# qzwlecr/p1

Measured on AMD Instinct MI355X. Metric: SHA-256 nonce-hashes/sec (GH/s), higher is better.
Workload: dtype u32

## Files before the change

p1_amd/csrc/p1hip.hip:

```cpp
#include <hip/hip_runtime.h>
#include <rccl/rccl.h>

#include <stdlib.h>
#include <string.h>

#include <algorithm>
#include <atomic>
#include <chrono>
#include <condition_variable>
#include <exception>
#include <mutex>
#include <string>
#include <thread>
#include <utility>
#include <vector>

#include "../../include/p1hip.h"
#include "async_slots.hpp"
#include "batch_plan.hpp"
#include "below_plan.hpp"
#include "belowb_plan.hpp"
#include "planner.hpp"
#include "scan_abi.hpp"
#include "scan_pack.hpp"
#include "tile_map.hpp"
#include "wide_plan.hpp"

extern "C" const unsigned char p1hip_kernels_co[];
extern "C" const unsigned char p1hip_batch_co[];
extern "C" const unsigned char p1hip_below_co[];
extern "C" const unsigned char p1hip_belowb_co[];

using namespace p1;

namespace {

thread_local std::string g_err;

int fail(int rc, const std::string& what) {
  g_err = what;
  return rc;
}

template <typename Fn>
int guarded(Fn&& fn) {
  try {
    return fn();
  } catch (const std::exception& ex) {
    return fail(P1HIP_ERR_HIP, std::string("host: ") + ex.what());
  } catch (...) {
    return fail(P1HIP_ERR_HIP, "host: unknown exception");
  }
}

#define HIPCHK(expr)                                                                        \
  do {                                                                                      \
    hipError_t e_ = (expr);                                                                 \
    if (e_ != hipSuccess)                                                                   \
      return fail(P1HIP_ERR_HIP, std::string(#expr) + ": " + hipGetErrorString(e_));       \
  } while (0)

#define NCCLCHK(expr)                                                                       \
  do {                                                                                      \
    ncclResult_t r_ = (expr);                                                               \
    if (r_ != ncclSuccess)                                                                  \
      return fail(P1HIP_ERR_RCCL, std::string(#expr) + ": " + ncclGetErrorString(r_));      \
  } while (0)

constexpr size_t kMaxKwTabs = 8;
constexpr uint64_t kMaxKwTabBytes = 8ull << 30;
constexpr uint64_t kMaxScanSpan = 1ull << 40;

enum KnobKind { kValue, kZeroDef, kFlag };
enum KnobWhen { kPerScan, kPerBatch, kAtInit };
enum KnobId {
  kSmallMaxNoncesKnob, kMaxLaunchBlocksKnob, kMaxScanSpanKnob, kKwtabMaxBytesKnob, kNoRcclKnob, kForceRcclKnob,
  kMinFastThreadsKnob, kTestFailDeviceKnob, kNoTableKnob, kNoSplitKnob, kScanGridKnob, kBatchMaxNoncesKnob,
  kBatchMaxTilesKnob, kWideMaxNoncesKnob, kWideMaxSegsKnob, kWideMinFastThreadsKnob, kBelowPathKnob,
  kBelowMaxSliceKnob, kKnobCount
};
struct Knob {
  const char* name;
  uint64_t def, max;
  KnobKind kind;
  KnobWhen when;
  const char* what;
};
const Knob kKnobs[] = {
    {"P1HIP_SMALL_MAX_NONCES", kSmallMaxNonces, kSmallMaxNonces, kValue, kPerScan,
     "shares of at most this many nonces take the one-launch small path; 0 turns it off, so small parity ranges "
     "run the fast kernel variants"},
    {"P1HIP_MAX_LAUNCH_BLOCKS", kMaxLaunchBlocks, kMaxLaunchBlocks, kZeroDef, kPerScan,
     "workgroups per k_scan launch, so GPU tests run the multi-launch path on small ranges; a larger piece gets "
     "a launch of its own (at most kMaxFastThreads / kBlock = 2^18 workgroups, far below HIP's grid limit)"},
    {"P1HIP_MAX_SCAN_SPAN", kMaxScanSpan, ~0ull, kZeroDef, kPerScan, "nonces per piece of a device's share"},
    {"P1HIP_KWTAB_MAX_BYTES", kMaxKwTabBytes, ~0ull, kValue, kPerScan,
     "MODE 5 table cap; a larger table re-plans the share without MODE 5"},
    {"P1HIP_NO_RCCL", 0, 1, kFlag, kAtInit,
     "combine the per-device results through the host, so the multi-device path (threads, sharding, combine) "
     "runs with the same GPU listed twice on a 1-GPU box"},
    {"P1HIP_FORCE_RCCL", 0, 1, kFlag, kAtInit, "a communicator even for one device"},
    {"P1HIP_MIN_FAST_THREADS", kMinFastThreads, ~0ull, kValue, kAtInit,
     "planner occupancy floor; 1 keeps k = 3 on small ranges so every k = 3 variant runs on the GPU"},
    {"P1HIP_TEST_FAIL_DEVICE", ~0ull, ~0ull, kValue, kAtInit,
     "device index whose scan phase reports a failure (the multi-device error path); default -1: none"},
    {"P1HIP_NO_TABLE", 0, 1, kFlag, kAtInit,
     "no MODE 5: layouts whose tail block 1 holds only lo digits run the digit-update variants (A/B, and a "
     "second kernel path to cross-check MODE 5)"},
    {"P1HIP_NO_SPLIT", 0, 1, kFlag, kAtInit,
     "straddling lo digits use mode 2 instead of the split modes (A/B builds with -DP1_NV2_PLAIN)"},
    {"P1HIP_SCAN_GRID", 0, kMaxLaunchBlocks, kZeroDef, kPerScan,
     "k_scan's grid instead of the device's workgroup slots (the default, 0); at or above a launch's tile count "
     "every workgroup runs one tile and the queue hands out none (the round-5 dispatch, same code object)"},
    {"P1HIP_BATCH_MAX_NONCES", kBatchMaxNonces, kBatchMaxNonces, kValue, kPerBatch,
     "requests of at most this many nonces are coalesced by p1hip_scan_batch; 0 runs every request "
     "individually; independent of P1HIP_SMALL_MAX_NONCES"},
    {"P1HIP_BATCH_MAX_TILES", kBatchMaxTiles, kBatchMaxTiles, kZeroDef, kPerBatch,
     "tiles per launch pair, so GPU tests run several launch pairs on small batches (batch_layout raises it to "
     "the largest single request's tile count)"},
    {"P1HIP_WIDE_MAX_NONCES", kWideMaxNonces, kWideMaxNonces, kValue, kPerBatch,
     "requests above the coalescing limit and of at most this many nonces share k_scan launches in "
     "p1hip_scan_batch_wide; larger ones run individually (0: all of them)"},
    {"P1HIP_WIDE_MAX_SEGS", kMaxSegs, kMaxSegs, kZeroDef, kPerBatch,
     "segments per k_scan launch of p1hip_scan_batch_wide, so GPU tests run many launches back to back on small "
     "calls and requests whose pieces land in different launches"},
    {"P1HIP_WIDE_MIN_FAST_THREADS", 0, ~0ull, kZeroDef, kPerBatch,
     "occupancy floor the wide requests are planned with instead of wide_min_fast_threads' rule (the default, "
     "0); 1 keeps k = 3"},
    {"P1HIP_BELOW_PATH", kBelowAuto, kBelowDense, kValue, kPerScan,
     "route of every slice of p1hip_scan_below: 0 chosen from the target (the default), 1 sparse (k_scan filters, "
     "the surviving tiles are marked), 2 dense (every nonce is marked), so GPU tests run both on one range"},
    {"P1HIP_BELOW_MAX_SLICE", 0, ~0ull, kZeroDef, kPerScan,
     "nonces per slice of p1hip_scan_below at the most, below the route's own limit, so GPU tests run several "
     "slices, with hits next to their edges, on small ranges"},
};
static_assert(sizeof kKnobs / sizeof kKnobs[0] == kKnobCount, "one row per KnobId, in its order");

bool test_knobs_on() {
  const char* m = getenv("P1HIP_TEST_KNOBS");
  return m && m[0] == '1' && m[1] == 0;
}

const char* test_knob(const char* name) {
  if (!test_knobs_on()) return nullptr;
  const char* v = getenv(name);
  return v && *v ? v : nullptr;
}

uint64_t knob(KnobId id) {
  const Knob& K = kKnobs[id];
  const char* v = test_knob(K.name);
  if (!v) return K.def;
  if (K.kind == kFlag) return v[0] == '1';
  const uint64_t n = strtoull(v, nullptr, 10);
  if (n == 0 && K.kind == kZeroDef) return K.def;
  return n < K.max ? n : K.max;
}

template <typename T, bool kPinned>
struct Buf {
  T* p = nullptr;
  size_t cap = 0;

  Buf() = default;
  Buf(const Buf&) = delete;
  Buf(Buf&& o) noexcept : p(std::exchange(o.p, nullptr)), cap(std::exchange(o.cap, 0)) {}
  Buf& operator=(Buf&& o) noexcept {
    if (this != &o) {
      (void)release();
      p = std::exchange(o.p, nullptr);
      cap = std::exchange(o.cap, 0);
    }
    return *this;
  }
  ~Buf() { (void)release(); }

  hipError_t release() {
    hipError_t e = hipSuccess;
    if (p) e = kPinned ? hipHostFree(p) : hipFree(p);
    p = nullptr;
    cap = 0;
    return e;
  }
  hipError_t reserve(size_t need, size_t floor, size_t extra = 0) {
    if (need <= cap) return hipSuccess;
    hipError_t e = release();
    if (e != hipSuccess) return e;
    size_t n = floor;
    while (n < need) n <<= 1;
    const size_t bytes = (n + extra) * sizeof(T);
    e = kPinned ? hipHostMalloc(&p, bytes, hipHostMallocDefault) : hipMalloc(&p, bytes);
    if (e != hipSuccess) p = nullptr;
    else cap = n;
    return e;
  }
};
template <typename T> using DevBuf = Buf<T, false>;
template <typename T> using PinnedBuf = Buf<T, true>;

struct SlotDev {
  DevBuf<BatchSeg> d_bseg;
  PinnedBuf<BatchSeg> h_bseg;
  DevBuf<uint32_t> d_btile0;
  PinnedBuf<uint32_t> h_btile0;
  DevBuf<Key> d_bout;
  PinnedBuf<Key> h_bout;
  DevBuf<Key> d_bpart;
  DevBuf<Key> d_part;
  DevBuf<Segment> d_seg;
  PinnedBuf<Segment> h_seg;
  DevBuf<BatchSeg> d_gseg;
  PinnedBuf<BatchSeg> h_gseg;
  DevBuf<WideRange> d_wrange;
  PinnedBuf<WideRange> h_wrange;
  DevBuf<uint32_t> d_wrange0;
  PinnedBuf<uint32_t> h_wrange0;
  DevBuf<Key> d_wout;
// ... 312 lines not shown

int run_small(Dev& d, const uint8_t* msg, size_t len, uint64_t lo, uint64_t hi, bool to_host, bool profiling,
              TileDump* dump = nullptr) {
  HIPCHK(hipSetDevice(d.ordinal));
  d.ctr = {};
  Plan plan;
  std::string err = make_plan(msg, len, lo, hi, plan, false);
  if (!err.empty()) return fail(P1HIP_ERR_ARGS, "planner: " + err);
  SmallArgs a;
  err = fill_small(plan, a, d.ctr);
  if (!err.empty()) return fail(P1HIP_ERR_ARGS, err);
  a.part = d.d_small_part.p;
  a.ticket = d.d_ticket.p;
  a.out_dev = d.d_res.p;
  a.out_host = to_host ? d.h_res.p : nullptr;
  int rc;
  if (dump) {
    dump->map = tile_map_small(plan);
    if ((rc = dump_poison(d, a.part, a.nblocks))) return rc;
  }
  size_t nev = 0;
  if (profiling && (rc = ev_record(d, nev))) return rc;
  HIPCHK(launch(d.f_small, a.nblocks, kBlock, d.stream, a));
  if (profiling && (rc = ev_record(d, nev))) return rc;
  if ((rc = ev_sum(d, nev))) return rc;
  return dump ? dump_collect(d, a.part, *dump) : P1HIP_OK;
}

constexpr int kNoTable = 1;

int kwtable_for(Dev& d, const Launch& L, uint64_t* dptr) {
  for (size_t i = 0; i < d.kwtabs.size(); ++i) {
    Dev::KwTab t = d.kwtabs[i];
    if (t.k == L.tabk && memcmp(t.w, L.tabw, sizeof t.w) == 0) {
      t.used_in = d.range_id;
      d.kwtabs.erase(d.kwtabs.begin() + (long)i);
      d.kwtabs.push_back(t);
      *dptr = (uint64_t)(uintptr_t)t.dptr;
      return P1HIP_OK;
    }
  }
  const size_t need = (size_t)pow10u(L.tabk) * 64u * sizeof(uint32_t);
  const size_t cap = (size_t)knob(kKwtabMaxBytesKnob);
  if (need > cap) return kNoTable;
  for (;;) {
    size_t held = 0;
    for (const Dev::KwTab& t : d.kwtabs) held += (size_t)pow10u(t.k) * 64u * sizeof(uint32_t);
    if (d.kwtabs.empty() || (d.kwtabs.size() < kMaxKwTabs && held + need <= cap)) break;
    size_t v = 0;
    while (v < d.kwtabs.size() && d.kwtabs[v].used_in == d.range_id) ++v;
    if (v == d.kwtabs.size()) return kNoTable;
    HIPCHK(hipFree(d.kwtabs[v].dptr));
    d.kwtabs.erase(d.kwtabs.begin() + (long)v);
  }
  Dev::KwTab t;
  memcpy(t.w, L.tabw, sizeof t.w);
  t.k = L.tabk;
  t.dptr = nullptr;
  t.used_in = d.range_id;
  const uint32_t rows = (uint32_t)pow10u(L.tabk);
  const hipError_t me = hipMalloc(&t.dptr, (size_t)rows * 64u * sizeof(uint32_t));
  if (me == hipErrorOutOfMemory) {
    (void)hipGetLastError();
    return kNoTable;
  }
  HIPCHK(me);
  KwTableArgs a;
  memset(&a, 0, sizeof a);
  memcpy(a.tabw, L.tabw, sizeof a.tabw);
  a.k = (uint32_t)L.tabk;
  a.qv = (uint32_t)(L.Y.q - 64);
  a.rows = rows;
  a.out = t.dptr;
  const hipError_t e = launch(d.f_kwtable, (rows + kBlock - 1) / kBlock, kBlock, d.stream, a);
  if (e != hipSuccess) {
    (void)hipFree(t.dptr);
    return fail(P1HIP_ERR_HIP, std::string("k_kwtable launch: ") + hipGetErrorString(e));
  }
  d.kwtabs.push_back(t);
  *dptr = (uint64_t)(uintptr_t)t.dptr;
  return P1HIP_OK;
}

uint32_t scan_grid_for(const Dev& d, uint32_t tiles) {
  const uint64_t g = knob(kScanGridKnob);
  return std::min(tiles, g > 0 ? (uint32_t)g : d.scan_grid);
}

int run_range(Dev& d, const uint8_t* msg, size_t len, uint64_t lo, uint64_t hi, bool profiling,
              uint64_t min_fast_threads, bool split, bool tabulate, TileDump* dump = nullptr, bool poison = true,
              bool collect = true) {
  HIPCHK(hipSetDevice(d.ordinal));
  d.range_id++;
  d.ctr = {};
  Plan plan;
  std::vector<uint64_t> tabptr;
  for (;;) {
    std::string err = make_plan(msg, len, lo, hi, plan, true, min_fast_threads, split, tabulate);
    if (!err.empty()) return fail(P1HIP_ERR_ARGS, "planner: " + err);
    tabptr.assign(plan.launches.size(), 0);
    bool replan = false;
    for (size_t i = 0; i < plan.launches.size() && !replan; ++i) {
      const Launch& L = plan.launches[i];
      if (!L.fast || (L.mode != 5 && L.mode != 7)) continue;
      const int rt = kwtable_for(d, L, &tabptr[i]);
      if (rt == kNoTable) replan = true;
      else if (rt != P1HIP_OK) return rt;
    }
    if (!replan) break;
    tabulate = false;
    d.replans++;
    plan = Plan();
  }
  const ScanPack P = pack_scan(plan, knob(kMaxLaunchBlocksKnob));
  HIPCHK(d.d_part.reserve(P.total_blocks, 1));
  HIPCHK(d.d_seg.reserve(P.batches.size() * kMaxSegs, 4 * kMaxSegs));
  HIPCHK(d.h_seg.reserve(P.batches.size() * kMaxSegs, 4 * kMaxSegs));
  int rc;
  if (dump) {
    dump->map = tile_map(plan, P);
    if (poison && (rc = dump_poison(d, d.d_part.p, P.total_blocks))) return rc;
  }
  size_t nev = 0;
  uint32_t part_off = 0;
  for (size_t bi = 0; bi < P.batches.size(); ++bi) {
    const ScanBatch& B = P.batches[bi];
    Segment* hs = d.h_seg.p + bi * kMaxSegs;
    Segment* ds = d.d_seg.p + bi * kMaxSegs;
    const std::string err = fill_segments(plan, P, B, tabptr.data(), hs, d.ctr);
    if (!err.empty()) return fail(P1HIP_ERR_ARGS, err);
    HIPCHK(hipMemcpyAsync(ds, hs, B.count * sizeof(Segment), hipMemcpyHostToDevice, d.stream));
    if (profiling && (rc = ev_record(d, nev))) return rc;
#ifdef P1_STATIC_GRID
    HIPCHK(launch(d.f_scan, B.blocks, kBlock, d.stream, (const Segment*)ds, (uint32_t)B.count,
                  (Key*)(d.d_part.p + part_off)));
#else
    HIPCHK(launch(d.f_scan, scan_grid_for(d, B.blocks), kBlock, d.stream, (const Segment*)ds,
                  (uint32_t)B.count, (Key*)(d.d_part.p + part_off), (uint32_t)B.blocks, d.d_scan_ticket.p));
#endif
    if (profiling && (rc = ev_record(d, nev))) return rc;
    part_off += B.blocks;
  }
  HIPCHK(launch(d.f_reduce, 1, kReduceThreads, d.stream, (const Key*)d.d_part.p, P.total_blocks, d.d_res.p));
  if ((rc = ev_sum(d, nev))) return rc;
  return dump && collect ? dump_collect(d, d.d_part.p, *dump) : P1HIP_OK;
}

int run_share(Dev& d, const uint8_t* msg, size_t len, uint64_t lo, uint64_t hi, const Runtime& R) {
  const uint64_t span = knob(kMaxScanSpanKnob);
  if (hi - lo < span)
    return run_range(d, msg, len, lo, hi, R.profiling, R.min_fast_threads, R.split, R.tabulate);
  Key best = {~0ull, ~0ull};
  ScanCounters sum;
  for (uint64_t a = lo;;) {
    const uint64_t b = hi - a < span ? hi : a + (span - 1);
    int r = run_range(d, msg, len, a, b, R.profiling, R.min_fast_threads, R.split, R.tabulate);
    if (r != P1HIP_OK) return r;
    Key k;
    HIPCHK(hipMemcpyAsync(&k, d.d_res.p, sizeof(Key), hipMemcpyDeviceToHost, d.stream));
    HIPCHK(hipStreamSynchronize(d.stream));
    if (key_lt(k, best)) best = k;
    sum += d.ctr;
    if (b == hi) break;
    a = b + 1;
  }
  d.ctr = sum;
  HIPCHK(hipMemcpyAsync(d.d_res.p, &best, sizeof(Key), hipMemcpyHostToDevice, d.stream));
  HIPCHK(hipStreamSynchronize(d.stream));
  return P1HIP_OK;
}

int scan_held(Runtime& R, const uint8_t* msg, size_t msg_len, uint64_t lower, uint64_t upper, uint64_t* out_hash,
              uint64_t* out_nonce) {
  const auto t0 = std::chrono::steady_clock::now();
  int rc = ensure_init(R);
  if (rc) return rc;
  Key res = {~0ull, 0};
  if (lower <= upper) {
    const size_t nd = R.devs.size();
    std::vector<uint64_t> slo(nd), shi(nd);
    std::vector<char> active(nd, 0);
    plan_shards(msg, msg_len, lower, upper, (int)nd, slo.data(), shi.data());
    for (size_t i = 0; i < nd; ++i) active[i] = slo[i] <= shi[i];
    std::vector<int> rcs(nd, 0);
    std::vector<std::string> errs(nd);
    auto run_threads = [&](auto&& fn) {
      if (nd == 1) {
        fn(0);
      } else {
        std::atomic<int> go{0};
        std::vector<std::thread> th;
        try {
          for (size_t i = 0; i < nd; ++i)
            th.emplace_back([&, i]() {
              while (go.load(std::memory_order_acquire) == 0) std::this_thread::yield();
              if (go.load(std::memory_order_acquire) == 1) fn(i);
            });
        } catch (...) {
          go.store(-1, std::memory_order_release);
          for (auto& t : th) t.join();
          throw;
        }
        go.store(1, std::memory_order_release);
        for (auto& t : th) t.join();
      }
    };
    auto run_phase = [&](double p1hip_device_stats_t::*ms, auto&& body) {
      run_threads([&](size_t i) {
        Dev& d = R.devs[i];
        const auto p0 = std::chrono::steady_clock::now();
        int r;
        try {
          r = body(i, d);
        } catch (const std::exception& ex) {
          try {
            r = fail(P1HIP_ERR_HIP, std::string("host: ") + ex.what());
          } catch (...) {
            r = P1HIP_ERR_HIP;
          }
        } catch (...) {
          r = P1HIP_ERR_HIP;
        }
// ... 168 lines not shown
    }
    if (Y.individual)
      for (size_t i = 0; i < n; ++i)
        if (q[i].lower <= q[i].upper && Y.tiles[i] == 0) {
          rc = scan_held(R, q[i].msg, q[i].len, q[i].lower, q[i].upper, &res[i].hash, &res[i].nonce);
          if (rc) return fail(rc, "request " + std::to_string(i) + ": " + g_err);
        }
    return P1HIP_OK;
  };
  if ((rc = run()) != P1HIP_OK) {
    const std::string keep = g_err;
    for (Dev& d : R.devs) (void)hipStreamSynchronize(d.stream);
    g_err = keep;
    return rc;
  }
  for (size_t i = 0; i < n; ++i) out[i] = res[i];
  R.bstats.calls++;
  R.bstats.requests += n;
  R.bstats.coalesced += Y.coalesced;
  R.bstats.individual += Y.individual;
  R.bstats.empty += Y.empty;
  R.bstats.launches += Y.launches.size();
  R.bstats.tiles += tiles;
  R.bstats.nonces += nonces;
  R.bstats.wall_ms += std::chrono::duration<double, std::milli>(std::chrono::steady_clock::now() - t0).count();
  return P1HIP_OK;
}

int scan_batch_locked(const p1hip_request_t* reqs, size_t n, p1hip_result_t* out) {
  Runtime& R = rt();
  std::lock_guard<std::mutex> g(R.mu);
  return scan_batch_held(R, reqs, n, out);
}

std::string wide_layout_held(const Runtime& R, const std::vector<BatchReq>& q, int ndev, WideLayout& Y) {
  const bool split = R.devs.empty() ? !knob(kNoSplitKnob) : R.split;
  return wide_layout(q.data(), q.size(), ndev, knob(kBatchMaxNoncesKnob), knob(kWideMaxNoncesKnob),
                     (uint32_t)knob(kWideMaxSegsKnob), knob(kWideMinFastThreadsKnob), split, Y);
}

int wide_reserve(Dev& d, const WideDevice& D) {
  const size_t nreq = D.reqs.size();
  HIPCHK(d.d_part.reserve(D.total_tiles, 1));
  HIPCHK(d.d_seg.reserve(D.fast.size(), 4 * kMaxSegs));
  HIPCHK(d.h_seg.reserve(D.fast.size(), 4 * kMaxSegs));
  HIPCHK(d.d_bseg.reserve(D.gsegs.size(), 64));
  HIPCHK(d.h_bseg.reserve(D.gsegs.size(), 64));
  HIPCHK(d.d_wrange.reserve(D.ranges.size(), 64));
  HIPCHK(d.h_wrange.reserve(D.ranges.size(), 64));
  HIPCHK(d.d_btile0.reserve(nreq, 64, 1));
  HIPCHK(d.h_btile0.reserve(nreq, 64, 1));
  HIPCHK(d.d_bout.reserve(nreq, 64));
  HIPCHK(d.h_bout.reserve(nreq, 64));
  return P1HIP_OK;
}

struct WideBufs {
  Key* d_part;
  Segment *d_seg, *h_seg;
  BatchSeg *d_gseg, *h_gseg;
  WideRange *d_range, *h_range;
  uint32_t *d_range0, *h_range0;
  Key *d_out, *h_out;
};

int wide_enqueue(Dev& d, const WideDevice& D, const WideBufs& b) {
  const size_t nreq = D.reqs.size();
  for (const WideLaunch& W : D.launches) {
    const std::string err = wide_fill_launch(D, W, b.h_seg + W.first);
    if (!err.empty()) return fail(P1HIP_ERR_ARGS, err);
  }
  if (!D.fast.empty())
    HIPCHK(hipMemcpyAsync(b.d_seg, b.h_seg, D.fast.size() * sizeof(Segment), hipMemcpyHostToDevice, d.stream));
  memcpy(b.h_range, D.ranges.data(), D.ranges.size() * sizeof(WideRange));
  memcpy(b.h_range0, D.req_range0.data(), (nreq + 1) * sizeof(uint32_t));
  HIPCHK(hipMemcpyAsync(b.d_range, b.h_range, D.ranges.size() * sizeof(WideRange), hipMemcpyHostToDevice, d.stream));
  HIPCHK(hipMemcpyAsync(b.d_range0, b.h_range0, (nreq + 1) * sizeof(uint32_t), hipMemcpyHostToDevice, d.stream));
  if (D.gen_tiles) {
    memcpy(b.h_gseg, D.gsegs.data(), D.gsegs.size() * sizeof(BatchSeg));
    HIPCHK(hipMemcpyAsync(b.d_gseg, b.h_gseg, D.gsegs.size() * sizeof(BatchSeg), hipMemcpyHostToDevice, d.stream));
    HIPCHK(launch(d.f_bscan, D.gen_tiles, kBlock, d.stream, (const BatchSeg*)b.d_gseg, (uint32_t)D.gsegs.size(),
                  (Key*)(b.d_part + D.gen_tile0)));
  }
  for (const WideLaunch& W : D.launches) {
#ifdef P1_STATIC_GRID
    HIPCHK(launch(d.f_scan, W.tiles, kBlock, d.stream, (const Segment*)(b.d_seg + W.first), (uint32_t)W.count,
                  (Key*)(b.d_part + W.tile0)));
#else
    HIPCHK(launch(d.f_scan, scan_grid_for(d, W.tiles), kBlock, d.stream, (const Segment*)(b.d_seg + W.first),
                  (uint32_t)W.count, (Key*)(b.d_part + W.tile0), (uint32_t)W.tiles, d.d_scan_ticket.p));
#endif
  }
  HIPCHK(launch(d.f_wreduce, (uint32_t)nreq, kBlock, d.stream, (const Key*)b.d_part, (const WideRange*)b.d_range,
                (const uint32_t*)b.d_range0, b.d_out));
  HIPCHK(hipMemcpyAsync(b.h_out, b.d_out, nreq * sizeof(Key), hipMemcpyDeviceToHost, d.stream));
  return P1HIP_OK;
}

int wide_enqueue(Dev& d, const WideDevice& D) {
  HIPCHK(hipSetDevice(d.ordinal));
  int rc = wide_reserve(d, D);
  if (rc) return rc;
  const WideBufs b = {d.d_part.p,   d.d_seg.p,    d.h_seg.p,    d.d_bseg.p, d.h_bseg.p, d.d_wrange.p,
                      d.h_wrange.p, d.d_btile0.p, d.h_btile0.p, d.d_bout.p, d.h_bout.p};
  return wide_enqueue(d, D, b);
}

int scan_batch_wide_locked(const p1hip_request_t* reqs, size_t n, p1hip_result_t* out) {
  Runtime& R = rt();
  std::lock_guard<std::mutex> g(R.mu);
  const auto t0 = std::chrono::steady_clock::now();
  int rc = ensure_init(R);
  if (rc) return rc;
  const std::vector<BatchReq> q = batch_reqs(reqs, n);
  WideLayout Y;
  const std::string lerr = wide_layout_held(R, q, (int)R.devs.size(), Y);
  if (!lerr.empty()) return fail(P1HIP_ERR_ARGS, lerr);
  std::vector<p1hip_result_t> res(n, p1hip_result_t{~0ull, 0});
  if (Y.small) {
    std::vector<p1hip_request_t> sq;
    std::vector<size_t> idx;
    for (size_t i = 0; i < n; ++i)
      if (Y.route[i] == kWideRouteSmall) {
        sq.push_back(reqs[i]);
        idx.push_back(i);
      }
    std::vector<p1hip_result_t> so(sq.size());
    if ((rc = scan_batch_held(R, sq.data(), sq.size(), so.data())) != P1HIP_OK) return rc;
    for (size_t j = 0; j < idx.size(); ++j) res[idx[j]] = so[j];
  }
  p1hip_wide_stats_t add{};
  auto run = [&]() -> int {
    for (size_t dv = 0; dv < Y.devs.size(); ++dv) {
      const WideDevice& D = Y.devs[dv];
      if (D.reqs.empty()) continue;
      if ((rc = wide_enqueue(R.devs[dv], D)) != P1HIP_OK) return rc;
      add.scan_launches += D.launches.size();
      add.scan_segments += D.fast.size();
      add.generic_launches += D.gen_tiles ? 1 : 0;
      add.generic_segments += D.gsegs.size();
      add.tiles += D.total_tiles;
      add.nonces += D.nonces;
    }
    for (size_t dv = 0; dv < Y.devs.size(); ++dv) {
      const WideDevice& D = Y.devs[dv];
      if (D.reqs.empty()) continue;
      Dev& d = R.devs[dv];
      HIPCHK(hipStreamSynchronize(d.stream));
      for (size_t r = 0; r < D.reqs.size(); ++r) {
        const Key kq = finish_key(d.h_bout.p[r]);
        res[D.reqs[r]] = p1hip_result_t{kq.h, kq.n};
      }
    }
    for (size_t i = 0; i < n; ++i)
      if (Y.route[i] == kWideRouteIndividual) {
        rc = scan_held(R, q[i].msg, q[i].len, q[i].lower, q[i].upper, &res[i].hash, &res[i].nonce);
        if (rc) return fail(rc, "request " + std::to_string(i) + ": " + g_err);
      }
    return P1HIP_OK;
  };
  if ((rc = run()) != P1HIP_OK) {
    const std::string keep = g_err;
    for (Dev& d : R.devs) (void)hipStreamSynchronize(d.stream);
    g_err = keep;
    return rc;
  }
  for (size_t i = 0; i < n; ++i) out[i] = res[i];
  p1hip_wide_stats_t& S = R.wstats;
  S.calls++;
  S.requests += n;
  S.empty += Y.empty;
  S.small += Y.small;
  S.wide += Y.wide;
  S.individual += Y.individual;
  S.scan_launches += add.scan_launches;
// ... 296 lines not shown
    HIPCHK(dn.reserve(n, n));
    HIPCHK(dp.reserve(blocks, blocks));
    HIPCHK(hipMemcpyAsync(dh.p, hashes, n * 8, hipMemcpyHostToDevice, d.stream));
    HIPCHK(hipMemcpyAsync(dn.p, nonces, n * 8, hipMemcpyHostToDevice, d.stream));
    HIPCHK(launch(d.f_pairs, blocks, kBlock, d.stream, (const uint64_t*)dh.p, (const uint64_t*)dn.p, (uint64_t)n,
                  dp.p));
    HIPCHK(launch(d.f_reduce, 1, kReduceThreads, d.stream, (const Key*)dp.p, blocks, d.d_res.p));
    HIPCHK(hipMemcpyAsync(d.h_res.p, d.d_res.p, sizeof(Key), hipMemcpyDeviceToHost, d.stream));
    HIPCHK(hipStreamSynchronize(d.stream));
    res = d.h_res.p[0];
  }
  res = finish_key(res);
  *out_hash = res.h;
  *out_nonce = res.n;
  return P1HIP_OK;
}

int scan_tiles_locked(const uint8_t* msg, size_t msg_len, uint64_t lower, uint64_t upper, size_t cap, size_t* count,
                      p1hip_tile_t* tiles, int* route, uint64_t* out_hash, uint64_t* out_nonce) {
  Runtime& R = rt();
  std::lock_guard<std::mutex> g(R.mu);
  int rc = ensure_init(R);
  if (rc) return rc;
  Dev& d = R.devs[0];
  d.replans = 0;
  TileDump dump;
  const bool small = upper - lower < knob(kSmallMaxNoncesKnob);
  rc = small ? run_small(d, msg, msg_len, lower, upper, false, R.profiling, &dump)
             : run_range(d, msg, msg_len, lower, upper, R.profiling, R.min_fast_threads, R.split, R.tabulate, &dump);
  if (rc) return rc;
  *count = dump.map.size();
  for (size_t i = 0; i < dump.map.size() && i < cap; ++i) {
    const TileInfo& T = dump.map[i];
    p1hip_tile_t& o = tiles[i];
    memset(&o, 0, sizeof o);
    o.launch = T.launch;
    o.tile = T.tile;
    o.kind = T.kind;
    o.k = T.k;
    o.nruns = T.nruns;
    for (uint32_t r = 0; r < T.nruns; ++r)
      o.runs[r] = {T.runs[r].first, T.runs[r].stride, T.runs[r].run_len, T.runs[r].count};
    o.hash = dump.part[i].h;
    o.nonce = dump.part[i].n;
  }
  *route = small ? 1 : 0;
  const Key res = finish_key(dump.res);
  *out_hash = res.h;
  *out_nonce = res.n;
  return P1HIP_OK;
}

static_assert(P1HIP_BELOW_MAX_SLICE == kBelowMaxSliceSparse && P1HIP_BELOW_MAX_SLICE_DENSE == kBelowMaxSliceDense &&
                  P1HIP_BELOW_DENSE_TARGET == kBelowDenseTarget,
              "p1hip.h and below_abi.hpp disagree");

int below_mark(Dev& d, const BelowTable& B, uint64_t target) {
  const size_t nseg = B.T.segs.size(), words = (size_t)B.tiles * kBelowWordsPerTile;
  HIPCHK(hipSetDevice(d.ordinal));
  HIPCHK(d.d_mseg.reserve(nseg, 64));
  HIPCHK(d.h_mseg.reserve(nseg, 64));
  HIPCHK(d.d_marks.reserve(words, 4096));
  HIPCHK(d.h_marks.reserve(words, 4096));
  memcpy(d.h_mseg.p, B.T.segs.data(), nseg * sizeof(BatchSeg));
  HIPCHK(hipMemcpyAsync(d.d_mseg.p, d.h_mseg.p, nseg * sizeof(BatchSeg), hipMemcpyHostToDevice, d.stream));
  HIPCHK(launch(d.f_mark, B.tiles, kBlock, d.stream, (const BatchSeg*)d.d_mseg.p, (uint32_t)nseg, target, d.d_marks.p));
  HIPCHK(hipMemcpyAsync(d.h_marks.p, d.d_marks.p, words * sizeof(uint64_t), hipMemcpyDeviceToHost, d.stream));
  HIPCHK(hipStreamSynchronize(d.stream));
  return P1HIP_OK;
}

int below_filter(Runtime& R, const uint8_t* msg, size_t msg_len, uint64_t lo, uint64_t hi, uint64_t target,
                 std::vector<BelowPiece>& pieces, std::vector<Key>& cand_part, p1hip_below_stats_t& add) {
  const size_t nd = R.devs.size();
  std::vector<uint64_t> slo(nd), shi(nd);
  plan_shards(msg, msg_len, lo, hi, (int)nd, slo.data(), shi.data());
  std::vector<TileDump> dumps(nd);
  int rc;
  for (size_t i = 0; i < nd; ++i) {
    if (slo[i] > shi[i]) continue;
    Dev& d = R.devs[i];
    d.replans = 0;
    if ((rc = run_range(d, msg, msg_len, slo[i], shi[i], R.profiling, R.min_fast_threads, R.split, R.tabulate,
                        &dumps[i], false, false)))
      return rc;
    add.scan_nonces += d.ctr.scan_nonces;
    d.acc.scan_launches += d.ctr.scan_launches;
    d.acc.scan_nonces += d.ctr.scan_nonces;
    d.acc.scan_alg_ops += d.ctr.scan_ops;
    d.acc.scan_kernel_ms += d.ctr.scan_ms;
  }
  for (size_t i = 0; i < nd; ++i) {
    if (slo[i] > shi[i]) continue;
    Dev& d = R.devs[i];
    HIPCHK(hipSetDevice(d.ordinal));
    if ((rc = dump_collect(d, d.d_part.p, dumps[i]))) return rc;
    for (size_t t = 0; t < dumps[i].map.size(); ++t)
      if (below_candidate(dumps[i].map[t], dumps[i].part[t], target)) {
        below_tile_pieces(dumps[i].map[t], (uint32_t)cand_part.size(), pieces);
        cand_part.push_back(dumps[i].part[t]);
      }
  }
  return P1HIP_OK;
}

int scan_below_held(Runtime& R, const uint8_t* msg, size_t msg_len, uint64_t lower, uint64_t upper, uint64_t target,
                    size_t cap, std::vector<p1hip_result_t>& res) {
  const auto t0 = std::chrono::steady_clock::now();
  int rc = ensure_init(R);
  if (rc) return rc;
  const int path = (int)knob(kBelowPathKnob);
  const uint64_t max_slice = knob(kBelowMaxSliceKnob);
  p1hip_below_stats_t add{};
  auto run = [&]() -> int {
    std::vector<BelowPiece> pieces;
    std::vector<Key> cand_part;
    std::vector<BelowHit> got;
    BelowTable B;
    for (uint64_t lo = lower;;) {
      const size_t want = cap - res.size();
      const BelowSlice S = below_next_slice(lo, upper, target, want, path, max_slice);
      pieces.clear();
      cand_part.clear();
      got.clear();
      if (S.dense) {
        below_dense_pieces(S.lo, S.hi, pieces);
        add.dense_slices++;
      } else {
        if ((rc = below_filter(R, msg, msg_len, S.lo, S.hi, target, pieces, cand_part, add))) return rc;
        add.sparse_slices++;
        add.candidate_tiles += cand_part.size();
      }
      for (size_t first = 0; first < pieces.size() && got.size() < (S.dense ? want : ~(size_t)0); first += B.count) {
        std::string err = below_build_table(msg, msg_len, pieces, first, B);
        if (!err.empty()) return fail(P1HIP_ERR_ARGS, err);
        if (B.count == 0 || B.tiles == 0) return fail(P1HIP_ERR_HIP, "internal: empty refine table");
        if ((rc = below_mark(R.devs[0], B, target))) return rc;
        add.mark_launches++;
        add.mark_nonces += B.T.nonces;
        err = below_decode(B, pieces, R.devs[0].h_marks.p, target, S.dense ? want - got.size() : ~(size_t)0, got);
        if (!err.empty()) return fail(P1HIP_ERR_HIP, err);
      }
      if (!S.dense) {
        const std::string err = below_check_candidates(cand_part, got);
        if (!err.empty()) return fail(P1HIP_ERR_HIP, err);
        below_sort_hits(got);
      }
      for (size_t i = 0; i < got.size() && res.size() < cap; ++i) res.push_back({got[i].key.h, got[i].key.n});
      add.slices++;
      add.examined += S.hi - S.lo + 1;
      if (res.size() == cap || S.hi == upper) return P1HIP_OK;
      lo = S.hi + 1;
    }
  };
  if ((rc = run()) != P1HIP_OK) {
    const std::string keep = g_err;
    for (Dev& d : R.devs) (void)hipStreamSynchronize(d.stream);
    g_err = keep;
    return rc;
  }
  p1hip_below_stats_t& T = R.lstats;
  T.calls++;
  T.slices += add.slices;
  T.sparse_slices += add.sparse_slices;
  T.dense_slices += add.dense_slices;
  T.examined += add.examined;
  T.scan_nonces += add.scan_nonces;
// ... 668 lines not shown
```

p1_amd/csrc/planner.hpp:

```cpp
#pragma once
#include <stdint.h>
#include <string.h>

#include <string>
#include <vector>

#include "scan_core.hpp"

namespace p1 {

constexpr uint64_t kMaxFastThreads = 1ull << 26;
constexpr uint64_t kMaxGenericThreads = 1ull << 26;
constexpr uint64_t kAlgOpsPerCompression = 1384;
constexpr uint64_t kMinFastThreads = 1ull << 18;
#ifndef P1_MAX_TAB_DIGITS
#define P1_MAX_TAB_DIGITS 7
#endif
constexpr int kMaxTabDigits = P1_MAX_TAB_DIGITS;

inline uint64_t pow10u(int e) {
  static constexpr uint64_t kPow10[20] = {1ull, 10ull, 100ull, 1000ull, 10000ull, 100000ull, 1000000ull, 10000000ull,
                                          100000000ull, 1000000000ull, 10000000000ull, 100000000000ull,
                                          1000000000000ull, 10000000000000ull, 100000000000000ull,
                                          1000000000000000ull, 10000000000000000ull, 100000000000000000ull,
// ... 10 lines not shown
  uint32_t r;
  uint64_t len;
};

inline void make_prefix(const uint8_t* msg, size_t L, Prefix& P) {
  for (int i = 0; i < 8; ++i) P.mid[i] = iv256(i);
  P.len = (uint64_t)L + 1;
  const uint64_t nfull = P.len / 64;
  uint8_t blk[64];
  for (uint64_t b = 0; b < nfull; ++b) {
    for (int j = 0; j < 64; ++j) {
      const uint64_t pos = b * 64 + j;
      blk[j] = pos < L ? msg[pos] : (uint8_t)' ';
    }
    uint32_t w[64];
    for (int t = 0; t < 16; ++t)
      w[t] = ((uint32_t)blk[4 * t] << 24) | ((uint32_t)blk[4 * t + 1] << 16) |
             ((uint32_t)blk[4 * t + 2] << 8) | (uint32_t)blk[4 * t + 3];
    compress_full(P.mid, w);
  }
  P.r = (uint32_t)(P.len % 64);
  memset(P.rem, 0, sizeof P.rem);
  for (uint32_t j = 0; j < P.r; ++j) {
    const uint64_t pos = nfull * 64 + j;
    P.rem[j] = pos < L ? msg[pos] : (uint8_t)' ';
  }
}

struct Layout {
  int d;
  int q;
  int nb;
  int vb;
  int k;
  bool trail;
  bool tab;
  bool two;
};

inline Layout make_layout(uint32_t r, int d, bool tabulate = true, bool two_level = true) {
  Layout Y;
  Y.d = d;
  Y.tab = tabulate;
  Y.two = false;
  Y.q = (int)r + d - 1;
  Y.nb = ((int)r + d + 9 <= 64) ? 1 : 2;
  if (Y.nb == 1) { Y.vb = 0; Y.k = 3; Y.trail = false; }
  else if (Y.q <= 63) { Y.vb = 0; Y.k = 3; Y.trail = true; }
  else if (tabulate && two_level && Y.q == 64 && d > 3) { Y.vb = 1; Y.k = 3; Y.trail = false; Y.two = true; }
  else if (tabulate && Y.q - 63 <= kMaxTabDigits) { Y.vb = 1; Y.k = Y.q - 63; Y.trail = false; }
  else if (Y.q - 64 >= 2) { Y.vb = 1; Y.k = 3; Y.trail = false; }
  else { Y.vb = 1; Y.k = Y.q - 63; Y.trail = false; }
  return Y;
}

inline void make_tmpl(const Prefix& P, int d, int zero_digits, uint32_t tmpl[32], int* nb_out) {
  uint8_t b[128];
  memset(b, 0, sizeof b);
  memcpy(b, P.rem, P.r);
  for (int i = 0; i < d; ++i) b[P.r + i] = (i >= d - zero_digits) ? (uint8_t)'0' : 0;
  b[P.r + d] = 0x80;
  const int nb = ((int)P.r + d + 9 <= 64) ? 1 : 2;
  const uint64_t bits = (P.len + (uint64_t)d) * 8u;
  for (int i = 0; i < 8; ++i) b[64 * nb - 1 - i] = (uint8_t)(bits >> (8 * i));
  for (int t = 0; t < 32; ++t)
    tmpl[t] = ((uint32_t)b[4 * t] << 24) | ((uint32_t)b[4 * t + 1] << 16) |
              ((uint32_t)b[4 * t + 2] << 8) | (uint32_t)b[4 * t + 3];
  *nb_out = nb;
}

struct Launch {
  bool fast;
  int fv, nv, mode;
  bool trail;
  FastArgs fa;
  GenArgs ga;
  uint64_t threads;
  uint32_t blocks;
  uint64_t nonces;
  int btail;
  Layout Y;
  uint32_t tabw[16];
  int tabk;
};

struct Plan {
  std::vector<Launch> launches;
  uint32_t total_blocks = 0;
  uint64_t total_nonces = 0;
};

inline void add_generic(const Prefix& P, const Layout& Y, uint64_t s, uint64_t e, Plan& plan) {
  uint64_t cur = s;
  for (;;) {
    const uint64_t left = e - cur;
    const uint64_t cnt = left >= kMaxGenericThreads ? kMaxGenericThreads : left + 1;
    Launch Ln;
    memset(&Ln, 0, sizeof Ln);
    Ln.fast = false;
    int nb = 0;
    memcpy(Ln.ga.mid, P.mid, sizeof P.mid);
    make_tmpl(P, Y.d, 0, Ln.ga.tmpl, &nb);
    Ln.ga.lo = cur;
    Ln.ga.count = cnt;
    Ln.ga.d = (uint32_t)Y.d;
    Ln.ga.p_last = (uint32_t)Y.q;
    Ln.ga.nb = (uint32_t)nb;
    Ln.threads = cnt;
    Ln.blocks = (uint32_t)((cnt + kBlock - 1) / kBlock);
    Ln.nonces = cnt;
    Ln.btail = nb;
    Ln.ga.part_off = plan.total_blocks;
    plan.total_blocks += Ln.blocks;
    plan.total_nonces += cnt;
    plan.launches.push_back(Ln);
    if (cnt == left + 1) break;
    cur += cnt;
  }
}

struct Variant {
  int fv, nv, mode;
};

inline Variant fast_variant(const Layout& Y, bool split = true) {
  const int qv = Y.q - 64 * Y.vb;
  Variant v;
  if (Y.two) {
    v.fv = 15;
    v.nv = 1;
    v.mode = 7;
    return v;
  }
  if (Y.tab && Y.vb == 1 && Y.q - 63 == Y.k) {
    v.fv = 0;
    v.nv = 1;
    v.mode = 5;
    return v;
  }
  v.fv = (qv - Y.k + 1) >> 2;
  v.nv = (qv >> 2) - v.fv + 1;
  v.mode = 1;
  if (v.nv == 2) v.mode = !split ? 2 : (Y.k >= 2 && ((qv - 1) >> 2) == v.fv) ? 4 : 3;
  else if (!Y.trail && ((qv - Y.k + 1) & 3) == 0) v.mode = 6;
  return v;
}

inline std::string add_fast(const Prefix& P, const Layout& Y, uint64_t hs, uint64_t he, Plan& plan,
                            bool split = true) {
  const int k = Y.k;
  const int qv = Y.q - 64 * Y.vb;
  const Variant var = fast_variant(Y, split);
  const int fv = var.fv, nv = var.nv;
  uint32_t tmpl[32];
  int nb = 0;
  make_tmpl(P, Y.d, k, tmpl, &nb);
  if (nb != Y.nb) return "internal: tail block count mismatch";
  const uint32_t* vw = tmpl + 16 * Y.vb;
  for (int i = fv + nv + 1; i < 16; ++i) {
    const bool is_len = (!Y.trail && i == 15);
    if (!is_len && vw[i] != 0u) return "internal: unexpected non-zero tail word";
  }
  if (k > 3 && var.mode != 5) return "internal: more than 3 lo digits outside MODE 5";
  uint32_t dlt[3][2] = {{0, 0}, {0, 0}, {0, 0}};
  if (var.mode == 7) {
    if (Y.q != 64 || k != 3) return "internal: MODE 7 layout";
// ... 25 lines not shown
  if (Y.trail) {
    uint32_t w[64];
    for (int i = 0; i < 16; ++i) w[i] = tmpl[16 + i];
    for (int t = 16; t < 64; ++t) w[t] = sched(w, t);
    for (int t = 0; t < 64; ++t) fa.kw2[t] = k256(t) + w[t];
  }
  fa.dh = (uint32_t)(Y.d - k);
  fa.p_last = (uint32_t)(Y.q - k);
  fa.pre = mode == 7 ? 0u : (uint32_t)Y.vb;
  fa.kpow = (uint32_t)pow10u(k);
  fa.nsub = (mode == 5 && k > 3) ? (uint32_t)pow10u(k - 3) : 1u;
  fa.n1 = k >= 2 ? 10u : 1u;
  fa.n2 = k >= 3 ? 10u : 1u;
  for (int s = 0; s < 2; ++s) {
    fa.du[s] = dlt[0][s];
    fa.dt[s] = dlt[1][s] - 10u * dlt[0][s];
    fa.dhd[s] = dlt[2][s] - 10u * dlt[1][s];
  }
  const uint64_t max_hi = kMaxFastThreads / fa.nsub;
  uint64_t cur = hs;
  for (;;) {
    const uint64_t left = he - cur;
    const uint64_t cnt = left >= max_hi ? max_hi : left + 1;
    Launch Ln;
    memset(&Ln, 0, sizeof Ln);
    Ln.fast = true;
    Ln.fv = fv;
    Ln.nv = nv;
    Ln.mode = mode;
    Ln.trail = Y.trail;
    Ln.fa = fa;
    Ln.fa.hi_first = cur;
    Ln.fa.nthreads = (uint32_t)cnt;
    Ln.threads = fa.nsub > 1 ? (cnt + 63) / 64 * 64 * fa.nsub : cnt;
    Ln.blocks = (uint32_t)((Ln.threads + kBlock - 1) / kBlock);
    Ln.nonces = cnt * fa.kpow;
    Ln.btail = Y.nb;
    Ln.Y = Y;
    if (mode == 5 || mode == 7) memcpy(Ln.tabw, tmpl + 16, sizeof Ln.tabw);
    Ln.tabk = mode == 5 ? k : mode == 7 ? 1 : 0;
    Ln.fa.part_off = plan.total_blocks;
    plan.total_blocks += Ln.blocks;
    plan.total_nonces += Ln.nonces;
    plan.launches.push_back(Ln);
    if (cnt == left + 1) break;
    cur += cnt;
  }
  return std::string();
}

inline std::vector<uint32_t> build_kwtable(const Launch& L) {
  const int k = L.tabk;
  const int qv = L.Y.q - 64;
  const uint32_t rows = (uint32_t)pow10u(k);
  std::vector<uint32_t> tab((size_t)rows * 64u);
  for (uint32_t c = 0; c < rows; ++c) kwtable_row(L.tabw, k, qv, c, tab.data() + (size_t)c * 64u);
  return tab;
}

inline std::string add_pieces(const Prefix& P, const Layout& Y, uint64_t s, uint64_t e, Plan& plan, bool split) {
  auto edge = [&](uint64_t a, uint64_t b) -> std::string {
    if (Y.k <= 3) {
      add_generic(P, Y, a, b, plan);
      return std::string();
    }
    return add_pieces(P, make_layout(P.r, Y.d, false), a, b, plan, split);
  };
  const uint64_t B = pow10u(Y.k);
  const uint64_t hs = s / B + (s % B != 0 ? 1u : 0u);
  bool have = true;
  uint64_t he = 0;
  if (e % B == B - 1) he = e / B;
  else if (e / B == 0) have = false;
  else he = e / B - 1;
  if (have && hs > he) have = false;
  if (!have) return edge(s, e);
  std::string err;
  if (hs * B > s && !(err = edge(s, hs * B - 1)).empty()) return err;
  if (!(err = add_fast(P, Y, hs, he, plan, split)).empty()) return err;
  if (e % B != B - 1) return edge((he + 1) * B, e);
  return std::string();
}

inline std::string make_plan(const uint8_t* msg, size_t L, uint64_t lower, uint64_t upper, Plan& plan,
                             bool fast_ok = true, uint64_t min_fast_threads = kMinFastThreads, bool split = true,
                             bool tabulate = true) {
  Prefix P;
  make_prefix(msg, L, P);
  plan = Plan();
  for (int d = 1; d <= 20; ++d) {
    const uint64_t dlo = (d == 1) ? 0u : pow10u(d - 1);
    const uint64_t dhi = (d == 20) ? ~0ull : pow10u(d) - 1u;
    const uint64_t s = lower > dlo ? lower : dlo;
    const uint64_t e = upper < dhi ? upper : dhi;
    if (s > e) continue;
    Layout Y = make_layout(P.r, d, tabulate);
    if (Y.k > 3 && (e - s) / 1000u + 1 < min_fast_threads) Y = make_layout(P.r, d, false);
    if (Y.two && (e - s) / 1000u + 1 < min_fast_threads) Y = make_layout(P.r, d, tabulate, false);
    if (Y.k <= 3)
      while (Y.k > 1 && (e - s) / pow10u(Y.k) + 1 < min_fast_threads) --Y.k;
    if (!fast_ok || d <= Y.k) {
      add_generic(P, Y, s, e, plan);
      continue;
    }
    std::string err = add_pieces(P, Y, s, e, plan, split);
    if (!err.empty()) return err;
  }
  return std::string();
}


constexpr double kCyclesA = 4.37, kCyclesB = 2.66;
constexpr double kUnhoistedCyclesPerBlock = 1600.0 * 3.6;

inline double variant_cycles(int fv, int mode, bool trail) {
#define P1_COST(FV, MODE, TR, A, B) \
  if (fv == FV && mode == MODE && trail == TR) return (A) * kCyclesA + (B) * kCyclesB;
#include "variant_cost.inc"
#undef P1_COST
  return 0.0;
}

inline double nonce_cycles(const Prefix& P, int d) {
  const Layout Y = make_layout(P.r, d);
  const double unhoisted = kUnhoistedCyclesPerBlock * Y.nb;
  if (d <= Y.k) return unhoisted;
  const Variant v = fast_variant(Y);
  double c = variant_cycles(v.fv, v.mode, Y.trail);
  if (c <= 0.0) c = 1384.0 * 3.6 * Y.nb;
  return c + unhoisted / (double)pow10u(Y.k > 3 ? 3 : Y.k);
}

inline void plan_shards(const uint8_t* msg, size_t L, uint64_t lower, uint64_t upper, int n, uint64_t* first,
                        uint64_t* last, double* cost = nullptr) {
  typedef unsigned __int128 u128;
  Prefix P;
  make_prefix(msg, L, P);
  struct Piece { uint64_t s, e; double c; };
  std::vector<Piece> pcs;
  double total = 0.0;
  for (int d = 1; d <= 20; ++d) {
    const uint64_t dlo = (d == 1) ? 0u : pow10u(d - 1);
    const uint64_t dhi = (d == 20) ? ~0ull : pow10u(d) - 1u;
    const uint64_t s = lower > dlo ? lower : dlo;
    const uint64_t e = upper < dhi ? upper : dhi;
    if (s > e) continue;
    const Piece pc = {s, e, nonce_cycles(P, d)};
    pcs.push_back(pc);
    total += ((double)(e - s) + 1.0) * pc.c;
  }
  std::vector<u128> cut((size_t)n + 1);
  cut[0] = lower;
  cut[n] = (u128)upper + 1u;
  size_t j = 0;
  double before = 0.0;
  for (int i = 1; i < n; ++i) {
    const double t = total * (double)i / (double)n;
    while (j < pcs.size() && before + ((double)(pcs[j].e - pcs[j].s) + 1.0) * pcs[j].c <= t) {
      before += ((double)(pcs[j].e - pcs[j].s) + 1.0) * pcs[j].c;
      ++j;
    }
    u128 x = cut[n];
    if (j < pcs.size()) {
      const double off = (t - before) / pcs[j].c;
      const uint64_t span = pcs[j].e - pcs[j].s;
      const uint64_t o = off <= 0.0 ? 0u : off >= (double)span ? span : (uint64_t)off;
      x = (u128)pcs[j].s + o;
    }
    if (x < cut[i - 1]) x = cut[i - 1];
    if (x > cut[n]) x = cut[n];
    cut[i] = x;
  }
  for (int i = 0; i < n; ++i) {
    if (cut[i] < cut[i + 1]) {
      first[i] = (uint64_t)cut[i];
      last[i] = (uint64_t)(cut[i + 1] - 1u);
    } else {
      first[i] = 1;
      last[i] = 0;
    }
    if (cost) {
      cost[i] = 0.0;
      if (first[i] > last[i]) continue;
      for (const Piece& pc : pcs) {
        const uint64_t s = pc.s > first[i] ? pc.s : first[i];
        const uint64_t e = pc.e < last[i] ? pc.e : last[i];
        if (s <= e) cost[i] += ((double)(e - s) + 1.0) * pc.c;
      }
    }
  }
// ... 4 lines not shown
```

p1_amd/csrc/scan_pack.hpp:

```cpp
#pragma once
#include <string.h>

#include <algorithm>
#include <string>
#include <vector>

#include "planner.hpp"
#include "scan_abi.hpp"

namespace p1 {

constexpr uint32_t kMaxSegs = 64;
constexpr uint32_t kMaxLaunchBlocks = 1u << 22;

inline bool has_variant(int fv, int mode, bool trail) {
#define P1_CASE(FV, MODE, TR) \
  if (fv == FV && mode == MODE && trail == TR) return true;
#include "fast_variants.inc"
#undef P1_CASE
  return false;
}

struct ScanCounters {
  uint64_t fast_launches = 0, fast_nonces = 0, fast_ops = 0, gen_launches = 0, gen_nonces = 0;
  uint64_t scan_launches = 0, scan_nonces = 0, scan_ops = 0;
  double scan_ms = 0.0;
  ScanCounters& operator+=(const ScanCounters& o) {
    fast_launches += o.fast_launches; fast_nonces += o.fast_nonces; fast_ops += o.fast_ops;
    gen_launches += o.gen_launches; gen_nonces += o.gen_nonces;
    scan_launches += o.scan_launches; scan_nonces += o.scan_nonces; scan_ops += o.scan_ops;
    scan_ms += o.scan_ms;
    return *this;
  }
};

struct ScanBatch {
  size_t first, count;
  uint32_t blocks;
};

struct ScanPack {
  std::vector<size_t> order;
  std::vector<ScanBatch> batches;
  uint32_t total_blocks = 0;
};

inline ScanPack pack_scan(const Plan& plan, uint64_t max_blocks, uint32_t max_segs = kMaxSegs) {
  ScanPack P;
  P.order.resize(plan.launches.size());
  for (size_t i = 0; i < P.order.size(); ++i) P.order[i] = i;
  auto weight = [&](size_t i) -> uint64_t {
    const Launch& L = plan.launches[i];
    return L.fast ? (uint64_t)(L.fa.kpow / L.fa.nsub) * (uint64_t)L.btail : (uint64_t)L.btail - 1;
  };
  std::stable_sort(P.order.begin(), P.order.end(), [&](size_t a, size_t b) { return weight(a) > weight(b); });
  uint64_t all_blocks = 0;
  for (const Launch& L : plan.launches) all_blocks += L.blocks;
  const uint64_t nlaunch = (all_blocks + max_blocks - 1) / max_blocks;
  const uint64_t target = nlaunch > 1 ? (all_blocks + nlaunch - 1) / nlaunch : max_blocks;
  for (size_t r = 0; r < P.order.size(); ++r) {
    const Launch& L = plan.launches[P.order[r]];
    const uint64_t cur = P.batches.empty() ? 0 : P.batches.back().blocks;
    if (P.batches.empty() || P.batches.back().count == max_segs || cur + (uint64_t)L.blocks > max_blocks ||
        (cur > 0 && cur + L.blocks / 2 > target && P.batches.size() < nlaunch))
      P.batches.push_back({r, 0, 0});
    P.batches.back().count++;
    P.batches.back().blocks += L.blocks;
    P.total_blocks += L.blocks;
  }
  return P;
}

inline std::string fill_segments(const Plan& plan, const ScanPack& P, const ScanBatch& B, const uint64_t* tabptr,
                                 Segment* segs, ScanCounters& c) {
  uint32_t block0 = 0;
  for (size_t j = 0; j < B.count; ++j) {
    const size_t i = P.order[B.first + j];
    const Launch& L = plan.launches[i];
    Segment& S = segs[j];
    memset(&S, 0, sizeof S);
    S.block0 = block0;
    block0 += L.blocks;
    if (L.fast) {
      if (!has_variant(L.fv, L.mode, L.trail)) return "no fast kernel variant";
      S.kind = variant_id(L.fv, L.mode, L.trail);
      S.fa = L.fa;
      if (L.mode == 5 || L.mode == 7) S.fa.kwtab = tabptr[i];
      c.fast_launches++;
      c.fast_nonces += L.nonces;
      c.fast_ops += L.nonces * kAlgOpsPerCompression * (uint64_t)L.btail;
    } else {
      S.kind = kGenericKind;
      S.ga = L.ga;
      c.gen_launches++;
      c.gen_nonces += L.nonces;
    }
    c.scan_nonces += L.nonces;
    c.scan_ops += L.nonces * kAlgOpsPerCompression * (uint64_t)L.btail;
  }
  c.scan_launches++;
  return "";
}

inline std::string fill_small(const Plan& plan, SmallArgs& a, ScanCounters& c) {
  if (plan.launches.size() > kSmallMaxSegs || plan.total_blocks > kSmallMaxBlocks)
    return "internal: small plan exceeds its argument block";
  memset(&a, 0, sizeof a);
  uint32_t block0 = 0;
  for (size_t i = 0; i < plan.launches.size(); ++i) {
    const Launch& L = plan.launches[i];
    a.ga[i] = L.ga;
    a.block0[i] = block0;
    block0 += L.blocks;
    c.gen_launches++;
    c.gen_nonces += L.nonces;
    c.scan_ops += L.nonces * kAlgOpsPerCompression * (uint64_t)L.btail;
  }
  a.nseg = (uint32_t)plan.launches.size();
  a.nblocks = block0;
  c.scan_launches++;
  c.scan_nonces += plan.total_nonces;
  return "";
}

}
```

Before: 53.61.

## Recut the heaviest fast launch into a drain tail of cheaper pieces

Adds a planner step that takes the heaviest eligible fast launch and moves its last grid-worth of threads (slots*kBlock) into a separately planned tail with one less k. The tail pieces are marked drain and packed last, so the persistent-grid queue ends on lighter work. This is meant to cut tail imbalance when the final wave of long tiles leaves workgroup slots idle. It also folds the launch code into a shared helper that now clears the ticket words before each launch. That adds a memset per launch and more segments per scan.

```diff
diff --git a/p1_amd/csrc/p1hip.hip b/p1_amd/csrc/p1hip.hip
--- a/p1_amd/csrc/p1hip.hip
+++ b/p1_amd/csrc/p1hip.hip
@@ -77,7 +77,7 @@
   kSmallMaxNoncesKnob, kMaxLaunchBlocksKnob, kMaxScanSpanKnob, kKwtabMaxBytesKnob, kNoRcclKnob, kForceRcclKnob,
   kMinFastThreadsKnob, kTestFailDeviceKnob, kNoTableKnob, kNoSplitKnob, kScanGridKnob, kBatchMaxNoncesKnob,
   kBatchMaxTilesKnob, kWideMaxNoncesKnob, kWideMaxSegsKnob, kWideMinFastThreadsKnob, kBelowPathKnob,
-  kBelowMaxSliceKnob, kKnobCount
+  kBelowMaxSliceKnob, kScanQueueKnob, kKnobCount
 };
 struct Knob {
   const char* name;
@@ -133,6 +133,10 @@
     {"P1HIP_BELOW_MAX_SLICE", 0, ~0ull, kZeroDef, kPerScan,
      "nonces per slice of p1hip_scan_below at the most, below the route's own limit, so GPU tests run several "
      "slices, with hits next to their edges, on small ranges"},
+    {"P1HIP_SCAN_QUEUE", 0, kMaxLaunchBlocks, kZeroDef, kPerScan,
+     "SLOTS[,DIRTY]: plan and launch p1hip_scan / p1hip_scan_tiles as on a device of SLOTS workgroup slots (drain "
+     "pieces, grid), so a scan of about a hundred tiles runs the queue and the drain pieces; DIRTY = 1 leaves the "
+     "ticket words non-zero after every launch, as a launch that did not finish would"},
 };
 static_assert(sizeof kKnobs / sizeof kKnobs[0] == kKnobCount, "one row per KnobId, in its order");
 
@@ -611,21 +615,50 @@
   return P1HIP_OK;
 }
 
-uint32_t scan_grid_for(const Dev& d, uint32_t tiles) {
+struct QueueKnob {
+  uint32_t slots = 0;
+  bool dirty = false;
+};
+QueueKnob queue_knob() {
+  QueueKnob K;
+  K.slots = (uint32_t)knob(kScanQueueKnob);
+  const char* v = test_knob(kKnobs[kScanQueueKnob].name);
+  if (!K.slots || !v) return QueueKnob();
+  if (const char* c = strchr(v, ',')) K.dirty = c[1] == '1';
+  return K;
+}
+
+uint32_t drain_slots_for(const Dev& d) {
+  const QueueKnob K = queue_knob();
+  return K.slots ? K.slots : d.scan_grid;
+}
+
+int launch_scan(Dev& d, const Segment* ds, uint32_t nseg, Key* part, uint32_t tiles) {
+  if (tiles == 0) return P1HIP_OK;
+#ifdef P1_STATIC_GRID
+  HIPCHK(launch(d.f_scan, tiles, kBlock, d.stream, ds, nseg, part));
+#else
+  const QueueKnob K = queue_knob();
   const uint64_t g = knob(kScanGridKnob);
-  return std::min(tiles, g > 0 ? (uint32_t)g : d.scan_grid);
+  const uint32_t slots = g > 0 ? (uint32_t)g : K.slots ? K.slots : d.scan_grid;
+  HIPCHK(hipMemsetAsync(d.d_scan_ticket.p, 0, 2 * sizeof(uint32_t), d.stream));
+  HIPCHK(launch(d.f_scan, std::min(tiles, slots), kBlock, d.stream, ds, nseg, part, tiles, d.d_scan_ticket.p));
+  if (K.dirty) HIPCHK(hipMemsetAsync(d.d_scan_ticket.p, 0xA5, 2 * sizeof(uint32_t), d.stream));
+#endif
+  return P1HIP_OK;
 }
 
 int run_range(Dev& d, const uint8_t* msg, size_t len, uint64_t lo, uint64_t hi, bool profiling,
               uint64_t min_fast_threads, bool split, bool tabulate, TileDump* dump = nullptr, bool poison = true,
-              bool collect = true) {
+              bool collect = true, bool drain = true) {
   HIPCHK(hipSetDevice(d.ordinal));
   d.range_id++;
   d.ctr = {};
   Plan plan;
   std::vector<uint64_t> tabptr;
   for (;;) {
-    std::string err = make_plan(msg, len, lo, hi, plan, true, min_fast_threads, split, tabulate);
+    std::string err = make_plan(msg, len, lo, hi, plan, true, min_fast_threads, split, tabulate,
+                                drain ? drain_slots_for(d) : 0u);
     if (!err.empty()) return fail(P1HIP_ERR_ARGS, "planner: " + err);
     tabptr.assign(plan.launches.size(), 0);
     bool replan = false;
@@ -660,13 +693,7 @@
     if (!err.empty()) return fail(P1HIP_ERR_ARGS, err);
     HIPCHK(hipMemcpyAsync(ds, hs, B.count * sizeof(Segment), hipMemcpyHostToDevice, d.stream));
     if (profiling && (rc = ev_record(d, nev))) return rc;
-#ifdef P1_STATIC_GRID
-    HIPCHK(launch(d.f_scan, B.blocks, kBlock, d.stream, (const Segment*)ds, (uint32_t)B.count,
-                  (Key*)(d.d_part.p + part_off)));
-#else
-    HIPCHK(launch(d.f_scan, scan_grid_for(d, B.blocks), kBlock, d.stream, (const Segment*)ds,
-                  (uint32_t)B.count, (Key*)(d.d_part.p + part_off), (uint32_t)B.blocks, d.d_scan_ticket.p));
-#endif
+    if ((rc = launch_scan(d, ds, (uint32_t)B.count, d.d_part.p + part_off, B.blocks))) return rc;
     if (profiling && (rc = ev_record(d, nev))) return rc;
     part_off += B.blocks;
   }
@@ -1001,15 +1028,8 @@
     HIPCHK(launch(d.f_bscan, D.gen_tiles, kBlock, d.stream, (const BatchSeg*)b.d_gseg, (uint32_t)D.gsegs.size(),
                   (Key*)(b.d_part + D.gen_tile0)));
   }
-  for (const WideLaunch& W : D.launches) {
-#ifdef P1_STATIC_GRID
-    HIPCHK(launch(d.f_scan, W.tiles, kBlock, d.stream, (const Segment*)(b.d_seg + W.first), (uint32_t)W.count,
-                  (Key*)(b.d_part + W.tile0)));
-#else
-    HIPCHK(launch(d.f_scan, scan_grid_for(d, W.tiles), kBlock, d.stream, (const Segment*)(b.d_seg + W.first),
-                  (uint32_t)W.count, (Key*)(b.d_part + W.tile0), (uint32_t)W.tiles, d.d_scan_ticket.p));
-#endif
-  }
+  for (const WideLaunch& W : D.launches)
+    if (int rc = launch_scan(d, b.d_seg + W.first, (uint32_t)W.count, b.d_part + W.tile0, W.tiles)) return rc;
   HIPCHK(launch(d.f_wreduce, (uint32_t)nreq, kBlock, d.stream, (const Key*)b.d_part, (const WideRange*)b.d_range,
                 (const uint32_t*)b.d_range0, b.d_out));
   HIPCHK(hipMemcpyAsync(b.h_out, b.d_out, nreq * sizeof(Key), hipMemcpyDeviceToHost, d.stream));
@@ -1472,7 +1492,7 @@
     Dev& d = R.devs[i];
     d.replans = 0;
     if ((rc = run_range(d, msg, msg_len, slo[i], shi[i], R.profiling, R.min_fast_threads, R.split, R.tabulate,
-                        &dumps[i], false, false)))
+                        &dumps[i], false, false, false)))
       return rc;
     add.scan_nonces += d.ctr.scan_nonces;
     d.acc.scan_launches += d.ctr.scan_launches;
diff --git a/p1_amd/csrc/planner.hpp b/p1_amd/csrc/planner.hpp
--- a/p1_amd/csrc/planner.hpp
+++ b/p1_amd/csrc/planner.hpp
@@ -116,6 +116,7 @@
   Layout Y;
   uint32_t tabw[16];
   int tabk;
+  bool drain;
 };
 
 struct Plan {
@@ -307,9 +308,64 @@
   return std::string();
 }
 
+inline bool has_variant(int fv, int mode, bool trail) {
+#define P1_CASE(FV, MODE, TR) \
+  if (fv == FV && mode == MODE && trail == TR) return true;
+#include "fast_variants.inc"
+#undef P1_CASE
+  return false;
+}
+
+constexpr uint32_t kDrainMinRounds = 4;
+
+inline void recut_drain(const Prefix& P, Plan& plan, uint32_t slots, bool split) {
+  if (slots == 0 || plan.total_blocks / slots < kDrainMinRounds) return;
+  const uint64_t cut = (uint64_t)slots * kBlock;
+  size_t pick = plan.launches.size();
+  uint64_t best = 0;
+  for (size_t i = 0; i < plan.launches.size(); ++i) {
+    const Launch& L = plan.launches[i];
+    if (!L.fast || L.mode == 5 || L.mode == 7 || L.fa.nsub != 1 || L.Y.k < 2 || L.fa.nthreads <= 2 * cut) continue;
+    const uint64_t w = (uint64_t)L.fa.kpow * (uint64_t)L.btail;
+    if (w >= best) { best = w; pick = i; }
+  }
+  if (pick == plan.launches.size()) return;
+  const Launch& C = plan.launches[pick];
+  const uint64_t keep = C.fa.nthreads - cut;
+  const uint64_t h0 = C.fa.hi_first + keep, h1 = C.fa.hi_first + C.fa.nthreads - 1;
+  Layout Y = C.Y;
+  --Y.k;
+  Plan tail;
+  if (!add_fast(P, Y, h0 * 10u, h1 * 10u + 9u, tail, split).empty()) return;
+  for (const Launch& L : tail.launches)
+    if (L.mode == 5 || L.mode == 7 || !has_variant(L.fv, L.mode, L.trail)) return;
+  Plan out;
+  auto push = [&](Launch L) {
+    (L.fast ? L.fa.part_off : L.ga.part_off) = out.total_blocks;
+    out.total_blocks += L.blocks;
+    out.total_nonces += L.nonces;
+    out.launches.push_back(L);
+  };
+  for (size_t i = 0; i < plan.launches.size(); ++i) {
+    Launch L = plan.launches[i];
+    if (i == pick) {
+      L.fa.nthreads = (uint32_t)keep;
+      L.threads = keep;
+      L.blocks = (uint32_t)((keep + kBlock - 1) / kBlock);
+      L.nonces = keep * L.fa.kpow;
+    }
+    push(L);
+  }
+  for (Launch L : tail.launches) {
+    L.drain = true;
+    push(L);
+  }
+  plan = out;
+}
+
 inline std::string make_plan(const uint8_t* msg, size_t L, uint64_t lower, uint64_t upper, Plan& plan,
                              bool fast_ok = true, uint64_t min_fast_threads = kMinFastThreads, bool split = true,
-                             bool tabulate = true) {
+                             bool tabulate = true, uint32_t drain_slots = 0) {
   Prefix P;
   make_prefix(msg, L, P);
   plan = Plan();
@@ -331,6 +387,7 @@
     std::string err = add_pieces(P, Y, s, e, plan, split);
     if (!err.empty()) return err;
   }
+  if (fast_ok) recut_drain(P, plan, drain_slots, split);
   return std::string();
 }
 
diff --git a/p1_amd/csrc/scan_pack.hpp b/p1_amd/csrc/scan_pack.hpp
--- a/p1_amd/csrc/scan_pack.hpp
+++ b/p1_amd/csrc/scan_pack.hpp
@@ -12,14 +12,6 @@
 
 constexpr uint32_t kMaxSegs = 64;
 constexpr uint32_t kMaxLaunchBlocks = 1u << 22;
-
-inline bool has_variant(int fv, int mode, bool trail) {
-#define P1_CASE(FV, MODE, TR) \
-  if (fv == FV && mode == MODE && trail == TR) return true;
-#include "fast_variants.inc"
-#undef P1_CASE
-  return false;
-}
 
 struct ScanCounters {
   uint64_t fast_launches = 0, fast_nonces = 0, fast_ops = 0, gen_launches = 0, gen_nonces = 0;
@@ -37,6 +29,7 @@
 struct ScanBatch {
   size_t first, count;
   uint32_t blocks;
+  uint32_t drain_blocks = 0;
 };
 
 struct ScanPack {
@@ -53,7 +46,10 @@
     const Launch& L = plan.launches[i];
     return L.fast ? (uint64_t)(L.fa.kpow / L.fa.nsub) * (uint64_t)L.btail : (uint64_t)L.btail - 1;
   };
-  std::stable_sort(P.order.begin(), P.order.end(), [&](size_t a, size_t b) { return weight(a) > weight(b); });
+  std::stable_sort(P.order.begin(), P.order.end(), [&](size_t a, size_t b) {
+    const bool da = plan.launches[a].drain, db = plan.launches[b].drain;
+    return da != db ? db : weight(a) > weight(b);
+  });
   uint64_t all_blocks = 0;
   for (const Launch& L : plan.launches) all_blocks += L.blocks;
   const uint64_t nlaunch = (all_blocks + max_blocks - 1) / max_blocks;
@@ -66,6 +62,7 @@
       P.batches.push_back({r, 0, 0});
     P.batches.back().count++;
     P.batches.back().blocks += L.blocks;
+    if (L.drain) P.batches.back().drain_blocks += L.blocks;
     P.total_blocks += L.blocks;
   }
   return P;
```

Result: no change. 53.57 (-0.1%).
